# Stansfash/nonstationary-precip

Hardware: AMD Instinct MI355X
Metric: dsvi_elbo_steps_per_sec (higher is better)
Workload: dtype f32; 1 GPU; 2-layer DSVI DeepGP (hidden 3->2 + last 2->1), M=1024, S=10, minibatch 4096 (global, split over the GPUs) of synthetic N=1e5 spatio-temporal grid; fwd+ELBO+bwd+Adam; M=1024, S=10, per_gpu_batch=4096, global_batch=4096, N=100000, parallelism=dp1, kzz_cholesky_dtype=f64, hipgraph=True

## Files before the change

### nonstationary-precip_amd/csrc/gemm_i8.hip

```cpp
#include <cstdlib>
#include "common.h"
#include "radial.h"

namespace {

#ifndef NSGP_I8_DMA
#define NSGP_I8_DMA 1
#endif
constexpr int I8_BM = 128, I8_BN = 64, I8_BK = 32;
constexpr int i8_walk(int sk) { return sk == 4 ? 2 : 1; }
constexpr int I8_SW = 5;

typedef int v4i __attribute__((ext_vector_type(4)));
typedef int v16i __attribute__((ext_vector_type(16)));

__global__ __launch_bounds__(256) void i8_slice_w_kernel(const double* __restrict__ W, int64_t M, int64_t Mp, int64_t KB,
                                                         signed char* __restrict__ Wd, double* __restrict__ wsc) {
    __shared__ double lds[4];
    const int64_t b = blockIdx.y, m = blockIdx.x;
    signed char* out = Wd + b * (int64_t)I8_SW * KB * 2 * Mp * 16;
    const int64_t plane = KB * 2 * Mp * 16;
    if (m >= M) {
        for (int64_t k = threadIdx.x; k < KB * 32; k += 256)
            for (int a = 0; a < I8_SW; ++a) out[a * plane + ((k >> 5) * 2 + ((k >> 4) & 1)) * Mp * 16 + m * 16 + (k & 15)] = 0;
        return;
    }
    const double* row = W + (b * M + m) * M;
    const auto nmax = [](double a, double c) { return (a > c || a != a) ? a : c; };
    double mx = 0.0;
    for (int64_t k = threadIdx.x; k <= m; k += 256) mx = nmax(fabs(row[k]), mx);
    for (int off = 32; off > 0; off >>= 1) mx = nmax(__shfl_xor(mx, off, 64), mx);
    if ((threadIdx.x & 63) == 0) lds[threadIdx.x >> 6] = mx;
    __syncthreads();
    mx = nmax(nmax(lds[0], lds[1]), nmax(lds[2], lds[3]));
    const bool fin = mx <= 1.7976931348623157e308;
    int e = 0;
    (void)frexp(fin ? mx : 0.0, &e);
    const double rs = (fin && mx > 0.0) ? ldexp(1.0, e) : 1.0;
    if (threadIdx.x == 0) wsc[b * M + m] = fin ? rs / 64.0 : __builtin_nan("");
    const double inv = 64.0 / rs;
    for (int64_t k = threadIdx.x; k < KB * 32; k += 256) {
        double t = (fin && k <= m && k < M) ? row[k] * inv : 0.0;
        const int64_t o = ((k >> 5) * 2 + ((k >> 4) & 1)) * Mp * 16 + m * 16 + (k & 15);
#pragma unroll
        for (int a = 0; a < I8_SW; ++a) {
            const double d = rint(t);
            out[a * plane + o] = (signed char)(int)d;
            t = (t - d) * 128.0;
        }
    }
}

struct I8Rbf {
    static __device__ __forceinline__ double eval(double r2) { return t_fexp<double>(-0.5 * r2); }
};
template <int NU2> struct I8Matern {
    static __device__ __forceinline__ double eval(double s) { return MaternRadial<NU2>::template eval<double>(s); }
};
template <typename Radial, int D, int SK>
__global__ __launch_bounds__(256) void i8_kzx_build_kernel(const float* __restrict__ Z, const float* __restrict__ x, int64_t sx,
                                                           const float* __restrict__ ls, const float* __restrict__ os,
                                                           int64_t M, int64_t n, int64_t np, int64_t KB,
                                                           signed char* __restrict__ Kd, double* __restrict__ ksc,
                                                           float* __restrict__ Kf) {
    const int64_t b = blockIdx.z, kb = blockIdx.y;
    const int64_t j = (int64_t)blockIdx.x * 256 + threadIdx.x;
    __shared__ double zs[32][D];
    __shared__ int bad;
    if (threadIdx.x == 0) bad = 0;
    if (threadIdx.x < 32 * D) {
        const int kk = threadIdx.x / D, d = threadIdx.x % D;
        const int64_t k = kb * 32 + kk;
        zs[kk][d] = k < M ? (double)Z[(b * M + k) * D + d] / (double)ls[b * D + d] : 0.0;
    }
    __syncthreads();
    const double osd = (double)os[b];
    bool fin = fabs(osd) <= 1.7976931348623157e308;
#pragma unroll
    for (int d = 0; d < D; ++d) fin = fin && fabs((double)ls[b * D + d]) <= 1.7976931348623157e308;
    int e = 0;
    (void)frexp(fin ? osd : 0.0, &e);
    const double cs = ldexp(1.0, e);
    const double sc = fin ? osd * 64.0 / cs : 0.0;
    if (j < np) {
        double xs[D];
#pragma unroll
        for (int d = 0; d < D; ++d) xs[d] = j < n ? (double)x[b * sx + j * D + d] / (double)ls[b * D + d] : 0.0;
        signed char* out = Kd + b * (int64_t)SK * KB * 2 * np * 16;
        const int64_t plane = KB * 2 * np * 16;
#pragma unroll
        for (int h = 0; h < 2; ++h) {
            int pk[SK][4] = {};
#pragma unroll
            for (int q = 0; q < 16; ++q) {
                const int kk = h * 16 + q;
                double r2 = 0.0;
#pragma unroll
                for (int d = 0; d < D; ++d) { const double df = zs[kk][d] - xs[d]; r2 = __builtin_fma(df, df, r2); }
                const bool in = j < n && kb * 32 + kk < M;
                const bool nan_e = in && r2 != r2;
                if (nan_e) bad = 1;
                const double ev = in ? Radial::eval(r2) : 0.0;
                const double evd = nan_e ? 0.0 : ev;
                if (Kf && in) Kf[(b * M + kb * 32 + kk) * n + j] = (float)(osd * ev);
                double t = sc * evd;
#pragma unroll
                for (int s = 0; s < SK; ++s) {
                    const double dg = rint(t);
                    pk[s][q >> 2] |= ((int)dg & 0xFF) << (8 * (q & 3));
                    t = (t - dg) * 128.0;
                }
            }
#pragma unroll
            for (int s = 0; s < SK; ++s) {
                v4i v = {pk[s][0], pk[s][1], pk[s][2], pk[s][3]};
                *reinterpret_cast<v4i*>(out + s * plane + (kb * 2 + h) * np * 16 + j * 16) = v;
            }
        }
    }
    __syncthreads();
    if (threadIdx.x == 0)
        ksc[(b * KB + kb) * gridDim.x + blockIdx.x] = (fin && !bad) ? cs / 64.0 : __builtin_nan("");
}

template <int P64, int SK, int LEV>
__global__ __launch_bounds__(256, 2) void i8_proj_kernel(const signed char* __restrict__ Wd, const double* __restrict__ wsc,
                                                         const signed char* __restrict__ Kd, const double* __restrict__ ksc,
                                                         const float* __restrict__ rv, int64_t M, int64_t n, int64_t Mp,
                                                         int64_t np, int64_t KB, int tiles_n, float* __restrict__ Y,
                                                         void* __restrict__ p0, void* __restrict__ p1, int part_rows) {
    extern __shared__ __attribute__((aligned(16))) unsigned char i8_smem[];
    constexpr int A_STAGE = I8_SW * 2 * I8_BM * 16, B_STAGE = SK * 2 * I8_BN * 16;
    unsigned char* As = i8_smem;
    unsigned char* Bs = i8_smem + 2 * A_STAGE;
    double* Ws = reinterpret_cast<double*>(i8_smem + 2 * (A_STAGE + B_STAGE));
    float* Rs = reinterpret_cast<float*>(Ws + I8_BM);
    double* red = reinterpret_cast<double*>(Rs + I8_BM);
    const int tid = threadIdx.x, lane = tid & 63, wave = __builtin_amdgcn_readfirstlane(tid >> 6);
    const int wm0 = (wave >> 1) * 64, wn0 = (wave & 1) * 32;
    const int64_t bb = blockIdx.y;
    const int tiles_m = (int)(Mp / I8_BM);
    constexpr int TW = i8_walk(SK);
    const int walks_n = (tiles_n + TW - 1) / TW;
    const int bm = tiles_m - 1 - (int)blockIdx.x / walks_n;
    const int bn0 = ((int)blockIdx.x % walks_n) * TW;
    const int ntile = TW == 1 ? 1 : __builtin_amdgcn_readfirstlane(tiles_n - bn0 < TW ? tiles_n - bn0 : TW);
    const int64_t m0 = (int64_t)bm * I8_BM, n00 = (int64_t)bn0 * I8_BN;
    int nkb = (int)((m0 + I8_BM) / I8_BK);
    if (nkb > KB) nkb = (int)KB;
    const signed char* Wb = Wd + bb * (int64_t)I8_SW * KB * 2 * Mp * 16;
    const signed char* Kb = Kd + bb * (int64_t)SK * KB * 2 * np * 16;
    const int64_t wplane = KB * 2 * Mp * 16, kplane = KB * 2 * np * 16;

    constexpr int NPB = (SK * 128 + 255) / 256;
    const signed char* ga[5];
    const signed char* gb[NPB];
    auto pieces = [&](int t) __attribute__((always_inline)) {
        int tv = tid;
        asm volatile("" : "+v"(tv));
#pragma unroll
        for (int j = 0; j < 5; ++j) {
            const int q = tv + 256 * j;
            const int a = q >> 8, h = (q >> 7) & 1, row = q & 127;
            ga[j] = Wb + a * wplane + (int64_t)h * Mp * 16 + (m0 + row) * 16;
        }
#pragma unroll
        for (int j = 0; j < NPB; ++j) {
            int q = tv + 256 * j;
            if (q >= SK * 128) q = SK * 128 - 1;
            const int s = q >> 7, h = (q >> 6) & 1, col = q & 63;
            gb[j] = Kb + s * kplane + (int64_t)h * np * 16 + (n00 + t * I8_BN + col) * 16;
        }
    };
    const int64_t astep = 2 * Mp * 16, bstep = 2 * np * 16;
#if NSGP_I8_DMA
    typedef const __attribute__((address_space(1))) void* gptr_t;
    typedef __attribute__((address_space(3))) void* lptr_t;
    auto dma = [&](int kb, int buf) __attribute__((always_inline)) {
#pragma unroll
        for (int j = 0; j < 5; ++j)
            __builtin_amdgcn_global_load_lds((gptr_t)(ga[j] + (int64_t)kb * astep),
                                             (lptr_t)(As + buf * A_STAGE + (wave * 64 + 256 * j) * 16), 16, 0, 0);
#pragma unroll
        for (int j = 0; j < NPB; ++j)
            if (wave * 64 + 256 * j < SK * 128)
                __builtin_amdgcn_global_load_lds((gptr_t)(gb[j] + (int64_t)kb * bstep),
                                                 (lptr_t)(Bs + buf * B_STAGE + (wave * 64 + 256 * j) * 16), 16, 0, 0);
    };
#endif
    v4i ra[5], rb[NPB];
    auto gload = [&](int kb) __attribute__((always_inline)) {
#pragma unroll
        for (int j = 0; j < 5; ++j) ra[j] = *reinterpret_cast<const v4i*>(ga[j] + (int64_t)kb * astep);
#pragma unroll
        for (int j = 0; j < NPB; ++j) rb[j] = *reinterpret_cast<const v4i*>(gb[j] + (int64_t)kb * bstep);
    };
    auto sstore = [&](int buf) __attribute__((always_inline)) {
#pragma unroll
        for (int j = 0; j < 5; ++j) *reinterpret_cast<v4i*>(As + buf * A_STAGE + (tid + 256 * j) * 16) = ra[j];
#pragma unroll
        for (int j = 0; j < NPB; ++j)
            if (tid + 256 * j < SK * 128) *reinterpret_cast<v4i*>(Bs + buf * B_STAGE + (tid + 256 * j) * 16) = rb[j];
    };

    const int wave_nkb = __builtin_amdgcn_readfirstlane((int)((m0 + wm0 + 64 + I8_BK - 1) / I8_BK));
    const int half = lane >> 5, lr = lane & 31;
    const int64_t gx = (np + 255) >> 8;
    const double* ksb = ksc + bb * KB * gx;
    const float* rvb = rv ? rv + bb * M : nullptr;
    auto stage0 = [&](int t) __attribute__((always_inline)) {
        pieces(t);
#if NSGP_I8_DMA
        dma(0, 0);
#else
        gload(0);
        sstore(0);
#endif
        return ksb[((n00 + t * I8_BN) >> 8) + (int64_t)(tid < nkb ? tid : nkb - 1) * gx];
    };
    double kslot = stage0(0);
    const int64_t prow = m0 + (tid & (I8_BM - 1)), crow = prow < M ? prow : M - 1;
    const double wload = wsc[bb * M + crow];
    const float rload = rvb ? rvb[crow] : 0.0f;
    const double wrow = prow < M ? wload : 0.0;
    const float rrow = prow < M ? rload : 0.0f;
    if (tid < I8_BM) { Ws[tid] = wrow; Rs[tid] = rrow; }
#pragma unroll 1
    for (int t = 0; t < ntile; ++t) {
    const int bn = bn0 + t;
    const int64_t n0 = (int64_t)bn * I8_BN;
    const double* ks = ksb + (n0 >> 8);
    v16i acc[LEV][2];
#pragma unroll
    for (int l = 0; l < LEV; ++l)
#pragma unroll
        for (int i = 0; i < 2; ++i)
#pragma unroll
            for (int r = 0; r < 16; ++r) acc[l][i][r] = 0;
#if NSGP_I8_DMA
    asm volatile("s_waitcnt vmcnt(0)" ::: "memory");
#endif
    const double kscale = __syncthreads_or(kslot != kslot) ? __builtin_nan("") : ks[0];
    if (t > 0) pieces(t);
    for (int kb = 0; kb < nkb; ++kb) {
        const int buf = kb & 1;
#if NSGP_I8_DMA
        if (kb + 1 < nkb) dma(kb + 1, buf ^ 1);
#else
        if (kb + 1 < nkb) gload(kb + 1);
#endif
        if (kb < wave_nkb) {
            v4i af[2][2], bf[SK];
#pragma unroll
            for (int s = 0; s < SK; ++s)
                bf[s] = *reinterpret_cast<const v4i*>(Bs + buf * B_STAGE + ((s * 2 + half) * I8_BN + wn0 + lr) * 16);
#pragma unroll
            for (int i = 0; i < 2; ++i)
                af[0][i] = *reinterpret_cast<const v4i*>(As + buf * A_STAGE + ((0 * 2 + half) * I8_BM + wm0 + 32 * i + lr) * 16);
#pragma unroll
            for (int a = 0; a < I8_SW; ++a) {
                if (a + 1 < I8_SW) {
#pragma unroll
                    for (int i = 0; i < 2; ++i)
                        af[(a + 1) & 1][i] = *reinterpret_cast<const v4i*>(
                            As + buf * A_STAGE + (((a + 1) * 2 + half) * I8_BM + wm0 + 32 * i + lr) * 16);
                }
#pragma unroll
                for (int s = 0; s < SK; ++s)
                    if (a + s < LEV) {
#pragma unroll
                        for (int i = 0; i < 2; ++i)
                            acc[a + s][i] = __builtin_amdgcn_mfma_i32_32x32x32_i8(af[a & 1][i], bf[s], acc[a + s][i], 0, 0, 0);
                    }
            }
        }
#if NSGP_I8_DMA
        asm volatile("s_waitcnt vmcnt(0)" ::: "memory");
#else
        if (kb + 1 < nkb) sstore(buf ^ 1);
#endif
        __syncthreads();
    }

    if (t + 1 < ntile) kslot = stage0(t + 1);
    double sdot = 0.0, ssq = 0.0;
    int64_t m0e = m0;
    asm volatile("" : "+s"(m0e));
    int lanee = lane, tide = tid;
    asm volatile("" : "+v"(lanee), "+v"(tide));
    const int halfe = lanee >> 5, lre = lanee & 31;
    const int64_t col = n0 + wn0 + lre;
#pragma unroll
    for (int i = 0; i < 2; ++i)
#pragma unroll
        for (int r = 0; r < 16; ++r) {
            const int lrow = wm0 + 32 * i + (r & 3) + 8 * (r >> 2) + 4 * halfe;
            const int64_t row = m0e + lrow;
            const double wr = Ws[lrow];
            const float rr = Rs[lrow];
            double v = (double)acc[LEV - 1][i][r];
#pragma unroll
            for (int l = LEV - 2; l >= 0; --l) v = __builtin_fma(v, 0.0078125, (double)acc[l][i][r]);
            const bool in = row < M && col < n;
            v *= (in ? wr : 0.0) * kscale;
            if (in) Y[(bb * M + row) * n + col] = (float)v;
            sdot += v * ((rvb && in) ? (double)rr : 0.0);
            ssq += v * v;
        }
    sdot += __shfl_xor(sdot, 32, 64);
    ssq += __shfl_xor(ssq, 32, 64);
    __syncthreads();
    if (lanee < 32) {
        red[(0 + (wave >> 1)) * I8_BN + wn0 + lanee] = sdot;
        red[(2 + (wave >> 1)) * I8_BN + wn0 + lanee] = ssq;
    }
    __syncthreads();
    if (tide < I8_BN && n0 + tide < n) {
        const int64_t o = (bb * part_rows + bm) * n + n0 + tide;
        const double d = red[tide] + red[I8_BN + tide], q = red[2 * I8_BN + tide] + red[3 * I8_BN + tide];
        if (P64) {
            if (p0) reinterpret_cast<double*>(p0)[o] = d;
            reinterpret_cast<double*>(p1)[o] = q;
        } else {
            if (p0) reinterpret_cast<float*>(p0)[o] = (float)d;
            reinterpret_cast<float*>(p1)[o] = (float)q;
        }
    }
    }
}

static inline int64_t i8_mp(int64_t M) { return cdiv64(M, I8_BM) * I8_BM; }
static inline int64_t i8_np(int64_t n) { return cdiv64(n, I8_BN) * I8_BN; }
static inline int64_t i8_kb(int64_t M) { return cdiv64(M, I8_BK); }

template <typename Radial>
int i8_kzx_build_launch(const float* Z, const float* x, int64_t sx, const float* ls, const float* os, int64_t batch, int64_t M,
                        int64_t n, int D, int planes, void* Kd, double* kscale, float* Kzx_f32, void* stream) {
    const int64_t np = i8_np(n), KB = i8_kb(M);
    dim3 grid((unsigned)cdiv64(np, 256), (unsigned)KB, (unsigned)batch);
    hipStream_t st = (hipStream_t)stream;
    signed char* kd = (signed char*)Kd;
#define NSGP_I8_BUILD(DD, SS) hipLaunchKernelGGL((i8_kzx_build_kernel<Radial, DD, SS>), grid, dim3(256), 0, st, Z, x, sx, ls, os, M, n, np, KB, kd, kscale, Kzx_f32)
    if (planes == 4) {
        switch (D) { case 1: NSGP_I8_BUILD(1, 4); break; case 2: NSGP_I8_BUILD(2, 4); break; case 3: NSGP_I8_BUILD(3, 4); break;
                     default: NSGP_I8_BUILD(4, 4); break; }
    } else {
        switch (D) { case 1: NSGP_I8_BUILD(1, 5); break; case 2: NSGP_I8_BUILD(2, 5); break; case 3: NSGP_I8_BUILD(3, 5); break;
                     default: NSGP_I8_BUILD(4, 5); break; }
    }
#undef NSGP_I8_BUILD
    return nsgp_launch_status();
}

}

extern "C" {

int nsgp_i8_supported(int64_t M) { return (M >= 1 && M <= 4096) ? 1 : 0; }
size_t nsgp_i8_w_planes_bytes(int64_t batch, int64_t M) {
    return (batch > 0 && M > 0) ? (size_t)(batch * I8_SW * i8_kb(M) * 2 * i8_mp(M) * 16) : 0;
}
size_t nsgp_i8_k_planes_bytes(int64_t batch, int64_t M, int64_t n, int planes) {
    return (batch > 0 && M > 0 && n > 0 && (planes == 4 || planes == 5)) ? (size_t)(batch * planes * i8_kb(M) * 2 * i8_np(n) * 16) : 0;
}
size_t nsgp_i8_tiles(int64_t M) { return M > 0 ? (size_t)cdiv64(M, I8_BM) : 0; }
size_t nsgp_i8_kscale_count(int64_t batch, int64_t M, int64_t n) {
    return (batch > 0 && M > 0 && n > 0) ? (size_t)(batch * i8_kb(M) * cdiv64(i8_np(n), 256)) : 0;
}

int nsgp_i8_slice_w_f64(const double* W, int64_t batch, int64_t M, void* Wd, double* wscale, void* stream) {
    if (!W) return -1; if (batch < 0) return -2; if (M < 0 || !nsgp_i8_supported(M > 0 ? M : 1)) return -3;
    if (!Wd) return -4; if (!wscale) return -5;
    if (batch == 0 || M == 0) return 0;
    if (batch > 65535) return -2;
    hipLaunchKernelGGL(i8_slice_w_kernel, dim3((unsigned)i8_mp(M), (unsigned)batch), dim3(256), 0, (hipStream_t)stream, W, M,
                       i8_mp(M), i8_kb(M), (signed char*)Wd, wscale);
    return nsgp_launch_status();
}

int nsgp_i8_rbf_build_f32(const float* Z, const float* x, int64_t x_batch_stride, const float* ls, const float* os,
                          int64_t batch, int64_t M, int64_t n, int D, int planes, void* Kd, double* kscale, float* Kzx_f32,
                          void* stream) {
    if (planes != 4 && planes != 5) return -10;
    if (!Z) return -1; if (!x) return -2; if (x_batch_stride < 0) return -3; if (!ls) return -4; if (!os) return -5;
    if (batch < 0) return -6; if (M < 0 || !nsgp_i8_supported(M > 0 ? M : 1)) return -7; if (n < 0) return -8;
    if (D < 1 || D > 4) return -9; if (!Kd) return -10; if (!kscale) return -11;
    if (batch == 0 || M == 0 || n == 0) return 0;
    if (batch > 65535 || i8_kb(M) > 65535) return -6;
    return i8_kzx_build_launch<I8Rbf>(Z, x, x_batch_stride, ls, os, batch, M, n, D, planes, Kd, kscale, Kzx_f32, stream);
}

int nsgp_i8_matern_build_f32(const float* Z, const float* x, int64_t x_batch_stride, const float* ls, const float* os,
                             int64_t batch, int64_t M, int64_t n, int D, int nu2, int planes, void* Kd, double* kscale,
                             float* Kzx_f32, void* stream) {
    if (!Z) return -1; if (!x) return -2; if (x_batch_stride < 0) return -3; if (!ls) return -4; if (!os) return -5;
    if (batch < 0) return -6; if (M < 0 || !nsgp_i8_supported(M > 0 ? M : 1)) return -7; if (n < 0) return -8;
    if (D < 1 || D > 4) return -9; if (nu2 != 1 && nu2 != 3 && nu2 != 5) return -10;
    if (planes != 4 && planes != 5) return -11; if (!Kd) return -12; if (!kscale) return -13;
    if (batch == 0 || M == 0 || n == 0) return 0;
    if (batch > 65535 || i8_kb(M) > 65535) return -6;
    switch (nu2) {
        case 1: return i8_kzx_build_launch<I8Matern<1>>(Z, x, x_batch_stride, ls, os, batch, M, n, D, planes, Kd, kscale, Kzx_f32, stream);
        case 3: return i8_kzx_build_launch<I8Matern<3>>(Z, x, x_batch_stride, ls, os, batch, M, n, D, planes, Kd, kscale, Kzx_f32, stream);
        default: return i8_kzx_build_launch<I8Matern<5>>(Z, x, x_batch_stride, ls, os, batch, M, n, D, planes, Kd, kscale, Kzx_f32, stream);
    }
}

int nsgp_svgp_tri_gemm_colstats_i8(const void* Wd, const double* wscale, const void* Kd, const double* kscale,
                                   int planes, const float* rowvec, int64_t batch, int64_t M, int64_t n, float* Y,
                                   void* part_dot, void* part_sq, int64_t part_rows, int partials_f64, void* stream) {
    if (planes != 4 && planes != 5) return -5;
    if (!Wd) return -1; if (!wscale) return -2; if (!Kd) return -3; if (!kscale) return -4;
    if (batch < 0) return -6; if (M < 0 || !nsgp_i8_supported(M > 0 ? M : 1)) return -7; if (n < 0) return -8;
    if (!Y) return -9; if (!part_sq) return -11; if (part_rows < cdiv64(M > 0 ? M : 1, I8_BM)) return -12;
    if (batch == 0 || M == 0 || n == 0) return 0;
    const int64_t Mp = i8_mp(M), np = i8_np(n), KB = i8_kb(M);
    const int64_t tiles_n = np / I8_BN, tiles = (Mp / I8_BM) * cdiv64(tiles_n, i8_walk(planes));
    if (tiles > 2147483647LL || batch > 65535) return -8;
    const size_t lds = 2 * (size_t)(I8_SW * 2 * I8_BM * 16 + planes * 2 * I8_BN * 16) + I8_BM * (sizeof(double) + sizeof(float)) +
                       4 * I8_BN * sizeof(double);
    hipStream_t st = (hipStream_t)stream;
    dim3 grid((unsigned)tiles, (unsigned)batch);
#define NSGP_I8_PROJ(PP, SS) hipLaunchKernelGGL((i8_proj_kernel<PP, SS, (SS == 5 ? 6 : 5)>), grid, dim3(256), lds, st, (const signed char*)Wd, wscale, \
        (const signed char*)Kd, kscale, rowvec, M, n, Mp, np, KB, (int)tiles_n, Y, part_dot, part_sq, (int)part_rows)
    if (planes == 4) { if (partials_f64) NSGP_I8_PROJ(1, 4); else NSGP_I8_PROJ(0, 4); }
    else { if (partials_f64) NSGP_I8_PROJ(1, 5); else NSGP_I8_PROJ(0, 5); }
#undef NSGP_I8_PROJ
    return nsgp_launch_status();
}

}
```

Before: 249.9 steps/s.

## Restructure int8 W slicing kernel to one wavefront per row with vectorized stores

The slicing kernel that splits the f64 Cholesky-derived W into int8 planes now assigns one 64-lane wavefront per row, eight rows per workgroup. Each lane holds 16 contiguous row elements in registers, computes the row max with wave shuffles only (no LDS or barrier), and packs 16 int8 digits per plane into a single 16-byte vector store. The old version did per-byte scattered stores and a block-wide reduction. It costs heavy register use (up to 64 doubles per lane for M up to 4096) and adds a template dispatch on KB.

```diff
diff --git a/nonstationary-precip_amd/csrc/gemm_i8.hip b/nonstationary-precip_amd/csrc/gemm_i8.hip
--- a/nonstationary-precip_amd/csrc/gemm_i8.hip
+++ b/nonstationary-precip_amd/csrc/gemm_i8.hip
@@ -14,40 +14,55 @@
 typedef int v4i __attribute__((ext_vector_type(4)));
 typedef int v16i __attribute__((ext_vector_type(16)));
 
-__global__ __launch_bounds__(256) void i8_slice_w_kernel(const double* __restrict__ W, int64_t M, int64_t Mp, int64_t KB,
-                                                         signed char* __restrict__ Wd, double* __restrict__ wsc) {
-    __shared__ double lds[4];
-    const int64_t b = blockIdx.y, m = blockIdx.x;
-    signed char* out = Wd + b * (int64_t)I8_SW * KB * 2 * Mp * 16;
+constexpr int I8_SLICE_ROWS = 8;
+template <int RPL>
+__global__ __launch_bounds__(64 * I8_SLICE_ROWS) void i8_slice_w_kernel(const double* __restrict__ W, int64_t M, int64_t Mp,
+                                                                        int64_t KB, signed char* __restrict__ Wd,
+                                                                        double* __restrict__ wsc) {
+    const int lane = threadIdx.x & 63;
+    const int64_t b = blockIdx.y, m = (int64_t)blockIdx.x * I8_SLICE_ROWS + (threadIdx.x >> 6);
     const int64_t plane = KB * 2 * Mp * 16;
-    if (m >= M) {
-        for (int64_t k = threadIdx.x; k < KB * 32; k += 256)
-            for (int a = 0; a < I8_SW; ++a) out[a * plane + ((k >> 5) * 2 + ((k >> 4) & 1)) * Mp * 16 + m * 16 + (k & 15)] = 0;
-        return;
-    }
+    signed char* out = Wd + b * (int64_t)I8_SW * plane + m * 16;
     const double* row = W + (b * M + m) * M;
+    double v[RPL][16];
+#pragma unroll
+    for (int q = 0; q < RPL; ++q) {
+        const int64_t k0 = ((int64_t)q * 64 + lane) * 16;
+#pragma unroll
+        for (int e = 0; e < 16; ++e) v[q][e] = (m < M && k0 + e <= m) ? row[k0 + e] : 0.0;
+    }
     const auto nmax = [](double a, double c) { return (a > c || a != a) ? a : c; };
     double mx = 0.0;
-    for (int64_t k = threadIdx.x; k <= m; k += 256) mx = nmax(fabs(row[k]), mx);
+#pragma unroll
+    for (int q = 0; q < RPL; ++q)
+#pragma unroll
+        for (int e = 0; e < 16; ++e) mx = nmax(fabs(v[q][e]), mx);
     for (int off = 32; off > 0; off >>= 1) mx = nmax(__shfl_xor(mx, off, 64), mx);
-    if ((threadIdx.x & 63) == 0) lds[threadIdx.x >> 6] = mx;
-    __syncthreads();
-    mx = nmax(nmax(lds[0], lds[1]), nmax(lds[2], lds[3]));
     const bool fin = mx <= 1.7976931348623157e308;
-    int e = 0;
-    (void)frexp(fin ? mx : 0.0, &e);
-    const double rs = (fin && mx > 0.0) ? ldexp(1.0, e) : 1.0;
-    if (threadIdx.x == 0) wsc[b * M + m] = fin ? rs / 64.0 : __builtin_nan("");
+    int ex = 0;
+    (void)frexp(fin ? mx : 0.0, &ex);
+    const double rs = (fin && mx > 0.0) ? ldexp(1.0, ex) : 1.0;
+    if (lane == 0 && m < M) wsc[b * M + m] = fin ? rs / 64.0 : __builtin_nan("");
     const double inv = 64.0 / rs;
-    for (int64_t k = threadIdx.x; k < KB * 32; k += 256) {
-        double t = (fin && k <= m && k < M) ? row[k] * inv : 0.0;
-        const int64_t o = ((k >> 5) * 2 + ((k >> 4) & 1)) * Mp * 16 + m * 16 + (k & 15);
-#pragma unroll
-        for (int a = 0; a < I8_SW; ++a) {
-            const double d = rint(t);
-            out[a * plane + o] = (signed char)(int)d;
-            t = (t - d) * 128.0;
-        }
+#pragma unroll
+    for (int q = 0; q < RPL; ++q) {
+        const int64_t run = (int64_t)q * 64 + lane;
+        if (run >= KB * 2) break;
+        v4i dg[I8_SW];
+#pragma unroll
+        for (int a = 0; a < I8_SW; ++a) dg[a] = v4i{0, 0, 0, 0};
+#pragma unroll
+        for (int e = 0; e < 16; ++e) {
+            double t = (fin && m < M && run * 16 + e <= m) ? v[q][e] * inv : 0.0;
+#pragma unroll
+            for (int a = 0; a < I8_SW; ++a) {
+                const double d = rint(t);
+                dg[a][e >> 2] |= (int)((unsigned)(unsigned char)(signed char)(int)d << (8 * (e & 3)));
+                t = (t - d) * 128.0;
+            }
+        }
+#pragma unroll
+        for (int a = 0; a < I8_SW; ++a) *reinterpret_cast<v4i*>(out + a * plane + run * Mp * 16) = dg[a];
     }
 }
 
@@ -373,8 +388,14 @@
     if (!Wd) return -4; if (!wscale) return -5;
     if (batch == 0 || M == 0) return 0;
     if (batch > 65535) return -2;
-    hipLaunchKernelGGL(i8_slice_w_kernel, dim3((unsigned)i8_mp(M), (unsigned)batch), dim3(256), 0, (hipStream_t)stream, W, M,
-                       i8_mp(M), i8_kb(M), (signed char*)Wd, wscale);
+    static_assert(I8_BM % I8_SLICE_ROWS == 0, "Mp is whole workgroups of rows");
+    const dim3 grid((unsigned)(i8_mp(M) / I8_SLICE_ROWS), (unsigned)batch), block(64 * I8_SLICE_ROWS);
+    if (i8_kb(M) * 2 <= 64)
+        hipLaunchKernelGGL(i8_slice_w_kernel<1>, grid, block, 0, (hipStream_t)stream, W, M, i8_mp(M), i8_kb(M),
+                           (signed char*)Wd, wscale);
+    else
+        hipLaunchKernelGGL(i8_slice_w_kernel<4>, grid, block, 0, (hipStream_t)stream, W, M, i8_mp(M), i8_kb(M),
+                           (signed char*)Wd, wscale);
     return nsgp_launch_status();
 }
 
```

New measurement: 249.6 steps/s. About the same (-0.1%).
